# sczhou/ProPainter

Measured on NVIDIA H100. Metric: inpainted frames/sec at 432x240x80f, higher is better.
Workload: dtype f32 (TF32 tensor-core products, fp32 accumulate)

## Files before the change

include/propainter_b200.h:

```cpp
#ifndef PROPAINTER_B200_H
#define PROPAINTER_B200_H
#include <stddef.h>
#include <stdint.h>
#include <cuda_runtime_api.h>

#ifdef __cplusplus
extern "C" {
#endif

#define PP_ABI_VERSION 2
int pp_abi_version(void);
const char* pp_error_string(int code);

int pp_corr_build(const float* fmap, int D, const int* idx1, const int* idx2, int n_pairs, float* lvl0, int h, int w,
                  cudaStream_t stream);
int pp_corr_pool_pyramid(float* const* levels, long planes, int h, int w, cudaStream_t stream);
int pp_corr_lookup(const float* const* levels, const float* coords, float* out, long n_pairs, int h, int w,
                   cudaStream_t stream);
int pp_corr_lookup_ldg(const float* const* levels, const float* coords, float* out, long n_pairs, int h, int w,
                       cudaStream_t stream);
int pp_corr_lookup_f16(const float* const* levels, const float* coords, void* out, int ld_out, long n_pairs, int h, int w,
                       cudaStream_t stream);
int pp_corr_lookup_ldg_f16(const float* const* levels, const float* coords, void* out, int ld_out, long n_pairs, int h, int w,
                           cudaStream_t stream);
// ... 54 lines not shown
int pp_window_mask(const float* pmask, int lt, int h, int w, int fh, int fw, int nwh, int nww, int* flags,
                   cudaStream_t stream);

typedef struct PPAttnParams {
  const float* qkv;
  const float* pool;
  const int* key_tok;
  const int* flags;
  float* out;
  int ld_qkv, ld_pool, ld_out;
  int t, NT, WN, NKO, NP, C;
  int kf_start, kf_step, nkf;
  float scale_log2;
} PPAttnParams;
int pp_sparse_window_attn(const PPAttnParams* prm, int n_windows, cudaStream_t stream);
int pp_sparse_window_attn_mma(const PPAttnParams* prm, int n_windows, cudaStream_t stream);
int pp_sparse_window_attn_f16(const PPAttnParams* prm, int n_windows, cudaStream_t stream);

size_t pp_ffn_overlap_add_workspace_bytes(int frames, int h, int w, int CH);
int pp_ffn_overlap_add(const float* Y, int ldy, float* Z, int ldz, int frames, int h, int w, int CH, void* workspace,
                       size_t ws_bytes, cudaStream_t stream);
int pp_ffn_overlap_add_f16(const void* Y, int ldy, void* Z, int ldz, int frames, int h, int w, int CH, void* workspace,
                           size_t ws_bytes, cudaStream_t stream);

int pp_pool_depthwise(const float* x, int ld_x, const float* w_taps, const float* bias, float* out, int n, int H, int W, int C,
                      int kh, int kw, cudaStream_t stream);
int pp_pool_depthwise_f16(const void* x, int ld_x, const float* w_taps, const float* bias, void* out, int n, int H, int W, int C,
                          int kh, int kw, cudaStream_t stream);
int pp_add_layernorm(const float* x, const float* delta, const float* gamma, const float* beta, float* x_out, float* y, long rows,
                     int C, float eps, cudaStream_t stream);
int pp_add_layernorm_f16(const float* x, const void* delta, int delta_f16, const float* gamma, const float* beta, float* x_out,
                         void* y, int y_f16, long rows, int C, float eps, cudaStream_t stream);

int pp_gru_gate(const float* zr, const float* bias, const float* pre, const float* net, int ld_net, float* z, float* rnet,
                int ld_r, long npix, int C, cudaStream_t stream);
int pp_gru_update(const float* q, const float* bias, const float* pre, const float* z, float* net, int ld_net, float* net_copy,
                  long npix, int C, cudaStream_t stream);
int pp_raft_pack_motion(const float* mot, int ld_mot, const float* bias, const float* flow, float* d0, float* d1, int ld,
                        long npix, cudaStream_t stream);
int pp_gru_gate_f16(const void* zr, const float* bias, const float* pre, const float* net, int ld_net, float* z, void* rnet,
                    int ld_r, long npix, int C, cudaStream_t stream);
int pp_gru_update_f16(const void* q, const float* bias, const float* pre, const float* z, float* net, int ld_net, void* h_img,
                      int ld_img, void* net_copy, long npix, int C, cudaStream_t stream);
int pp_raft_pack_motion_f16(const void* mot, int ld_mot, const float* bias, const float* flow, void* d0, void* d1, int ld,
                            long npix, cudaStream_t stream);
int pp_raft_pack_motion_n(const float* mot, int ld_mot, const float* bias, const float* flow, float* d0, float* d1, int ld,
                          long npix, int cmot, cudaStream_t stream);

int pp_bias_act(const float* x, int ld_x, const float* bias, const float* res, int ld_res, float* out, int ld_out, long n_pix,
                int C, int act, float slope, int post_relu, cudaStream_t stream);
int pp_bias_act_pre(const float* x, int ld_x, const float* bias, const float* pre, int ld_pre, const float* res, int ld_res,
                    float* out, int ld_out, long n_pix, int C, int act, float slope, int post_relu, cudaStream_t stream);
int pp_bias_act_f16(const void* x, int ld_x, int x_f16, const float* bias, const float* pre, int ld_pre, const float* res, int ld_res,
                    void* out, int ld_out, int out_f16, long n_pix, int C, int act, float slope, int post_relu, cudaStream_t stream);

size_t pp_instance_norm_workspace_bytes(int n, long HW, int C);
int pp_instance_norm(const float* x, const float* res, float* out, int n, long HW, int C, float eps, int relu, int post_relu,
                     void* workspace, size_t ws_bytes, cudaStream_t stream);
int pp_upsample2x_bilinear(const float* src, float* dst, int n, int h, int w, int C, cudaStream_t stream);

int pp_mask_dilate(const uint8_t* src, float* dst, int T, int H, int W, int iterations, cudaStream_t stream);
int pp_u8_to_frames(const uint8_t* src, float* dst, int T, int H, int W, cudaStream_t stream);
int pp_resample_coeffs_bicubic(int in_size, int out_size, int* bounds, int* kk, long kk_capacity);
int pp_resample_index_nearest(int in_size, int out_size, int* idx);
int pp_resample_coeffs_linear_cv(int in_size, int out_size, int horizontal, int* ofs, short* coef);
size_t pp_resize_u8_bicubic_workspace_bytes(int T, int H, int Wo);
int pp_resize_u8_bicubic(const uint8_t* src, uint8_t* dst, int T, int H, int W, int Ho, int Wo, const int* bounds_x, const int* kk_x,
                         int ksize_x, const int* bounds_y, const int* kk_y, int ksize_y, void* workspace, size_t ws_bytes,
                         cudaStream_t stream);
int pp_resize_u8_nearest(const uint8_t* src, uint8_t* dst, int T, int H, int W, int Ho, int Wo, int C, const int* idx_x, const int* idx_y,
                         cudaStream_t stream);
int pp_resize_u8_bilinear_cv(const uint8_t* src, uint8_t* dst, int T, int H, int W, int Ho, int Wo, const int* xofs, const short* alpha,
                             const int* yofs, const short* beta, cudaStream_t stream);
int pp_resample_coeffs_linear_f32(int in_size, int out_size, int horizontal, int* ofs, float* coef);
int pp_resize_flow_linear_cv(const float* src, float* dst, int N, int H, int W, int Ho, int Wo, const int* xofs, const float* alpha,
                             const int* yofs, const float* beta, cudaStream_t stream);
#define PP_MAX_WINDOW 32
typedef struct PPWindowIds { int n; int frame[PP_MAX_WINDOW]; int first[PP_MAX_WINDOW]; } PPWindowIds;
int pp_composite_blend_u8(const float* pred, const float* masks, const uint8_t* ori, uint8_t* comp,
                          const PPWindowIds* ids, int H, int W, cudaStream_t stream);
int pp_composite_blend_f32(const float* pred, const float* masks, const uint8_t* ori, float* comp,
                           const PPWindowIds* ids, int H, int W, cudaStream_t stream);
// ... 19 lines not shown
```

propainter_b200/_lib.py:

```python
import ctypes
import os

_HERE = os.path.dirname(os.path.abspath(__file__))
LIB_PATH = os.environ.get("PROPAINTER_B200_LIB") or os.path.join(_HERE, "libpropainter_b200.so")

c_void_p, c_int, c_long, c_float, c_size_t = ctypes.c_void_p, ctypes.c_int, ctypes.c_long, ctypes.c_float, ctypes.c_size_t

PP_MAX_WINDOW = 32


class PPAttnParams(ctypes.Structure):
    _fields_ = [("qkv", c_void_p), ("pool", c_void_p), ("key_tok", c_void_p), ("flags", c_void_p), ("out", c_void_p),
                ("ld_qkv", c_int), ("ld_pool", c_int), ("ld_out", c_int),
                ("t", c_int), ("NT", c_int), ("WN", c_int), ("NKO", c_int), ("NP", c_int), ("C", c_int),
                ("kf_start", c_int), ("kf_step", c_int), ("nkf", c_int), ("scale_log2", c_float)]


PP_CONV_MAX_SEG = 4


class PPConvSeg(ctypes.Structure):
    _fields_ = [("x", c_void_p), ("ld", c_int), ("C", c_int)]


# ... 62 lines not shown
    "pp_gru_update": (c_int, [c_void_p, c_void_p, c_void_p, c_void_p, c_void_p, c_int, c_void_p, c_long, c_int, c_void_p]),
    "pp_raft_pack_motion": (c_int, [c_void_p, c_int, c_void_p, c_void_p, c_void_p, c_void_p, c_int, c_long, c_void_p]),
    "pp_gru_gate_f16": (c_int, [c_void_p, c_void_p, c_void_p, c_void_p, c_int, c_void_p, c_void_p, c_int, c_long, c_int, c_void_p]),
    "pp_gru_update_f16": (c_int, [c_void_p, c_void_p, c_void_p, c_void_p, c_void_p, c_int, c_void_p, c_int, c_void_p, c_long, c_int,
                                  c_void_p]),
    "pp_raft_pack_motion_f16": (c_int, [c_void_p, c_int, c_void_p, c_void_p, c_void_p, c_void_p, c_int, c_long, c_void_p]),
    "pp_raft_pack_motion_n": (c_int, [c_void_p, c_int, c_void_p, c_void_p, c_void_p, c_void_p, c_int, c_long, c_int, c_void_p]),
    "pp_bias_act": (c_int, [c_void_p, c_int, c_void_p, c_void_p, c_int, c_void_p, c_int, c_long, c_int, c_int, c_float, c_int,
                            c_void_p]),
    "pp_bias_act_pre": (c_int, [c_void_p, c_int, c_void_p, c_void_p, c_int, c_void_p, c_int, c_void_p, c_int, c_long, c_int, c_int, c_float,
                                c_int, c_void_p]),
    "pp_bias_act_f16": (c_int, [c_void_p, c_int, c_int, c_void_p, c_void_p, c_int, c_void_p, c_int, c_void_p, c_int, c_int, c_long, c_int,
                                c_int, c_float, c_int, c_void_p]),
    "pp_pool_depthwise": (c_int, [c_void_p, c_int, c_void_p, c_void_p, c_void_p, c_int, c_int, c_int, c_int, c_int, c_int, c_void_p]),
    "pp_add_layernorm": (c_int, [c_void_p, c_void_p, c_void_p, c_void_p, c_void_p, c_void_p, c_long, c_int, c_float, c_void_p]),
    "pp_pool_depthwise_f16": (c_int, [c_void_p, c_int, c_void_p, c_void_p, c_void_p, c_int, c_int, c_int, c_int, c_int, c_int,
                                      c_void_p]),
    "pp_add_layernorm_f16": (c_int, [c_void_p, c_void_p, c_int, c_void_p, c_void_p, c_void_p, c_void_p, c_int, c_long, c_int,
                                     c_float, c_void_p]),
    "pp_instance_norm_workspace_bytes": (c_size_t, [c_int, c_long, c_int]),
    "pp_instance_norm": (c_int, [c_void_p, c_void_p, c_void_p, c_int, c_long, c_int, c_float, c_int, c_int, c_void_p, c_size_t,
                                 c_void_p]),
    "pp_upsample2x_bilinear": (c_int, [c_void_p, c_void_p, c_int, c_int, c_int, c_int, c_void_p]),
    "pp_mask_dilate": (c_int, [c_void_p, c_void_p, c_int, c_int, c_int, c_int, c_void_p]),
    "pp_u8_to_frames": (c_int, [c_void_p, c_void_p, c_int, c_int, c_int, c_void_p]),
    "pp_resample_coeffs_bicubic": (c_int, [c_int, c_int, c_void_p, c_void_p, c_long]),
    "pp_resample_index_nearest": (c_int, [c_int, c_int, c_void_p]),
    "pp_resample_coeffs_linear_cv": (c_int, [c_int, c_int, c_int, c_void_p, c_void_p]),
    "pp_resize_u8_bicubic_workspace_bytes": (c_size_t, [c_int, c_int, c_int]),
    "pp_resize_u8_bicubic": (c_int, [c_void_p, c_void_p, c_int, c_int, c_int, c_int, c_int, c_void_p, c_void_p, c_int, c_void_p, c_void_p,
                                     c_int, c_void_p, c_size_t, c_void_p]),
    "pp_resize_u8_nearest": (c_int, [c_void_p, c_void_p, c_int, c_int, c_int, c_int, c_int, c_int, c_void_p, c_void_p, c_void_p]),
    "pp_resize_u8_bilinear_cv": (c_int, [c_void_p, c_void_p, c_int, c_int, c_int, c_int, c_int, c_void_p, c_void_p, c_void_p, c_void_p,
                                         c_void_p]),
    "pp_composite_blend_u8": (c_int, [c_void_p, c_void_p, c_void_p, c_void_p, ctypes.POINTER(PPWindowIds), c_int, c_int,
                                      c_void_p]),
    "pp_composite_blend_f32": (c_int, [c_void_p, c_void_p, c_void_p, c_void_p, ctypes.POINTER(PPWindowIds), c_int, c_int,
                                       c_void_p]),
    "pp_resample_coeffs_linear_f32": (c_int, [c_int, c_int, c_int, c_void_p, c_void_p]),
    "pp_resize_flow_linear_cv": (c_int, [c_void_p, c_void_p] + [c_int] * 5 + [c_void_p] * 5),
    "pp_extrapolate_u8": (c_int, [c_void_p, c_void_p, c_void_p, c_void_p] + [c_int] * 9 + [c_void_p]),
    "pp_mask_overlay_u8": (c_int, [c_void_p, c_void_p, c_void_p, c_int, c_int, c_int, c_void_p]),
    "pp_flow_maxrad": (c_int, [c_void_p, c_void_p] + [c_int] * 5 + [ctypes.c_float, c_void_p]),
    "pp_flow_to_image_u8": (c_int, [c_void_p, c_void_p, c_void_p] + [c_int] * 5 + [ctypes.c_float, c_int, c_void_p]),
    "pp_i3d_input": (c_int, [c_void_p, c_int, c_void_p, c_int, c_int, c_int, c_int, c_void_p]),
    "pp_maxpool3d_same": (c_int, [c_void_p, c_int, c_void_p, c_int] + [c_int] * 11 + [c_void_p]),
# ... 27 lines not shown
```

propainter_b200/csrc/gather_kernels.cu:

```cuda
#include <stdlib.h>
#include "pp_elem.cuh"
#include "pp_mma.cuh"
#include "../../include/propainter_b200.h"

#define PP_LAUNCH_CHECK() do { if (cudaPeekAtLastError() != cudaSuccess) return PP_ERR_LAUNCH; } while (0)

static inline int pp_blocks(long n, int per) { return (int)((n + per - 1) / per); }

__global__ void __launch_bounds__(256) k_imgprop_step(int H, int W, const float* __restrict__ cur,
    const float* __restrict__ mcur, const float* __restrict__ prev, const float* __restrict__ mprev,
    const float* __restrict__ fprop, const float* __restrict__ fcheck, float* __restrict__ out,
    float* __restrict__ mout, int nearest) {
  int pix = blockIdx.x * blockDim.x + threadIdx.x;
  if (pix < H * W) pp_imgprop_pixel(pix, H, W, cur, mcur, prev, mprev, fprop, fcheck, out, mout, nearest);
}

extern "C" size_t pp_img_prop_scan_workspace_bytes(int t, int H, int W) {
  return (size_t)t * 4 * H * W * sizeof(float);
}

extern "C" int pp_img_prop_scan(const float* frames, const float* flows_f, const float* flows_b,
                                const float* masks, float* out_frames, float* out_masks, void* workspace,
                                size_t ws_bytes, int t, int H, int W, int nearest, cudaStream_t stream) {
  if (t < 1 || H < 2 || W < 2) return PP_ERR_SHAPE;
// ... 412 lines not shown
  if (ws_bytes < pp_ffn_overlap_add_workspace_bytes(frames, h, w, CH)) return PP_ERR_WORKSPACE;
  float* F = (float*)workspace;
  const long n1 = (long)h * w * (CH / 4), n2 = (long)fh * fw * 49 * (CH / 4);
  if (n2 > 0x7fffffffL) return PP_ERR_SHAPE;
  k_ffn_fold_gelu<T><<<dim3(pp_blocks(n1, 256), frames), 256, 0, stream>>>(Y, ldy, CH, fh, fw, h, w, F);
  k_ffn_unfold<T><<<dim3(pp_blocks(n2, 256), frames), 256, 0, stream>>>(F, CH, fh, fw, h, w, Z, ldz);
  PP_LAUNCH_CHECK();
  return PP_OK;
}
extern "C" int pp_ffn_overlap_add(const float* Y, int ldy, float* Z, int ldz, int frames, int h, int w, int CH,
                                  void* workspace, size_t ws_bytes, cudaStream_t stream) {
  if (ldy < 49 * CH || ldz < 49 * CH || frames < 1 || frames > 65535) return PP_ERR_SHAPE;
  if (CH % 4 || ldy % 4 || ldz % 4) return PP_ERR_ALIGN;
  return pp_ffn_launch(Y, ldy, Z, ldz, frames, h, w, CH, workspace, ws_bytes, stream);
}
extern "C" int pp_ffn_overlap_add_f16(const void* Y, int ldy, void* Z, int ldz, int frames, int h, int w, int CH,
                                      void* workspace, size_t ws_bytes, cudaStream_t stream) {
  if (ldy < 49 * CH || ldz < 49 * CH || frames < 0 || frames > 65535) return PP_ERR_SHAPE;
  if (CH % 4 || ldy % 8 || ldz % 8 || ((uintptr_t)Y & 15) || ((uintptr_t)Z & 15) || ((uintptr_t)workspace & 15)) return PP_ERR_ALIGN;
  if (frames == 0 || h <= 0 || w <= 0) return PP_OK;
  return pp_ffn_launch((const __half*)Y, ldy, (__half*)Z, ldz, frames, h, w, CH, workspace, ws_bytes, stream);
}

template <typename TX, typename TO>
__global__ void __launch_bounds__(256) k_bias_act(const TX* x, int ld_x, const float* __restrict__ bias, const float* res,
                                                  int ld_res, TO* out, int ld_out, long n_pix, int C, int act, float slope,
                                                  int post_relu, const float* __restrict__ pre = nullptr, int ld_pre = 0) {
  const int c4n = C >> 2;
  const long i = (long)blockIdx.x * blockDim.x + threadIdx.x;
  if (i >= n_pix * c4n) return;
  const long pix = i / c4n; const int c = (int)(i - pix * c4n) * 4;
  const float4 v = pp_ld4(x + pix * ld_x + c);
  float r[4] = {v.x, v.y, v.z, v.w};
  if (bias != nullptr) {
    const float4 b = *reinterpret_cast<const float4*>(bias + c);
    r[0] += b.x; r[1] += b.y; r[2] += b.z; r[3] += b.w;
  }
  if (pre != nullptr) {
    const float4 b = *reinterpret_cast<const float4*>(pre + pix * ld_pre + c);
    r[0] += b.x; r[1] += b.y; r[2] += b.z; r[3] += b.w;
  }
#pragma unroll
  for (int k = 0; k < 4; ++k) {
    float t = r[k];
    if (act == 1) t = fmaxf(t, 0.f);
    else if (act == 2) t = t > 0.f ? t : t * slope;
// ... 135 lines not shown
#pragma unroll
      for (int e = 0; e < 4; ++e) y[e] = fmaxf(y[e], 0.f);
    }
    *reinterpret_cast<float4*>(out + off) = make_float4(y[0], y[1], y[2], y[3]);
  }
}
extern "C" size_t pp_instance_norm_workspace_bytes(int n, long HW, int C) {
  return (size_t)n * pp_in_splits(n, HW) * 2 * C * sizeof(float);
}
extern "C" int pp_instance_norm(const float* x, const float* res, float* out, int n, long HW, int C, float eps, int relu,
                                int post_relu, void* workspace, size_t ws_bytes, cudaStream_t stream) {
  if (C % 4 || ((uintptr_t)x & 15) || ((uintptr_t)out & 15) || ((uintptr_t)res & 15) || ((uintptr_t)workspace & 15)) return PP_ERR_ALIGN;
  if (C < 4 || C > 512 || n < 1 || n > 65535 || HW < 1) return PP_ERR_SHAPE;
  if (ws_bytes < pp_instance_norm_workspace_bytes(n, HW, C)) return PP_ERR_WORKSPACE;
  const int S = pp_in_splits(n, HW);
  const int chunk = (int)((HW + S - 1) / S);
  float* part = (float*)workspace;
  k_inorm_stats<<<dim3(S, n), 256, 0, stream>>>(x, HW, C, chunk, S, part);
  k_inorm_apply<<<dim3(S, n), 256, 0, stream>>>(x, part, S, res, out, HW, C, chunk, eps, relu, post_relu);
  PP_LAUNCH_CHECK();
  return PP_OK;
}

__global__ void __launch_bounds__(256) k_upsample2x(const float* __restrict__ src, float* __restrict__ dst, int n, int h,
                                                    int w, int C) {
  const int c4n = C >> 2, H = 2 * h, W = 2 * w;
  const long i = (long)blockIdx.x * blockDim.x + threadIdx.x;
  if (i >= (long)n * H * W * c4n) return;
  const int c = (int)(i % c4n) * 4; const long px = i / c4n;
  const int b = (int)(px / ((long)H * W)); const int r = (int)(px - (long)b * H * W); const int y = r / W, x = r - y * W;
  const PPUp uy = pp_up2_coord(y, h), ux = pp_up2_coord(x, w);
  const float* p = src + (((long)b * h + uy.i0) * w + ux.i0) * C + c;
  const float4 v00 = *reinterpret_cast<const float4*>(p), v01 = *reinterpret_cast<const float4*>(p + (long)ux.step * C);
  const float4 v10 = *reinterpret_cast<const float4*>(p + (long)uy.step * w * C);
  const float4 v11 = *reinterpret_cast<const float4*>(p + ((long)uy.step * w + ux.step) * C);
  float4 o;
  o.x = pp_up2_blend(v00.x, v01.x, v10.x, v11.x, uy, ux); o.y = pp_up2_blend(v00.y, v01.y, v10.y, v11.y, uy, ux);
  o.z = pp_up2_blend(v00.z, v01.z, v10.z, v11.z, uy, ux); o.w = pp_up2_blend(v00.w, v01.w, v10.w, v11.w, uy, ux);
  reinterpret_cast<float4*>(dst)[i] = o;
}
extern "C" int pp_upsample2x_bilinear(const float* src, float* dst, int n, int h, int w, int C, cudaStream_t stream) {
  if (C % 4) return PP_ERR_ALIGN;
  if (h < 2 || w < 2) return PP_ERR_SHAPE;
  const long total = (long)n * 4 * h * w * (C / 4);
  k_upsample2x<<<pp_blocks(total, 256), 256, 0, stream>>>(src, dst, n, h, w, C);
  PP_LAUNCH_CHECK();
  return PP_OK;
}

template <typename T>
__global__ void __launch_bounds__(256) k_gru_gate(const T* __restrict__ zr, const float* __restrict__ bias,
    const float* __restrict__ pre, const float* __restrict__ net, int ld_net, float* __restrict__ z, T* __restrict__ rnet,
    int ld_r, long npix, int C) {
  const int c4n = C >> 2;
  const long i = (long)blockIdx.x * blockDim.x + threadIdx.x;
  if (i >= npix * c4n) return;
  const long pix = i / c4n; const int c = (int)(i - pix * c4n) * 4;
  float4 zv = pp_ld4(zr + pix * 2 * C + c), rv = pp_ld4(zr + pix * 2 * C + C + c);
  float4 bz = make_float4(0.f, 0.f, 0.f, 0.f), br = bz;
  if (bias != nullptr) { bz = *reinterpret_cast<const float4*>(bias + c); br = *reinterpret_cast<const float4*>(bias + C + c); }
  if (pre != nullptr) {
    const float4 pz = *reinterpret_cast<const float4*>(pre + pix * 2 * C + c), pr = *reinterpret_cast<const float4*>(pre + pix * 2 * C + C + c);
    zv.x += pz.x; zv.y += pz.y; zv.z += pz.z; zv.w += pz.w; rv.x += pr.x; rv.y += pr.y; rv.z += pr.z; rv.w += pr.w;
  }
  const float4 h = *reinterpret_cast<const float4*>(net + pix * ld_net + c);
  float4 zo, ro;
  zo.x = 1.0f / (1.0f + expf(-(zv.x + bz.x))); zo.y = 1.0f / (1.0f + expf(-(zv.y + bz.y)));
  zo.z = 1.0f / (1.0f + expf(-(zv.z + bz.z))); zo.w = 1.0f / (1.0f + expf(-(zv.w + bz.w)));
// ... 445 lines not shown
```

propainter_b200/model/modules/sparse_transformer.py:

```python
import torch
import torch.nn.functional as F

from ... import config, ops
from ...nn_util import as_nchw, as_pm, cl, conv
from ...window_index import padded_grid, token_grid, window_key_table

WIN = (5, 9)
POOL = (4, 4)
KS, ST, PD = 7, 3, 3


class TransformerExec:
    def __init__(self, net, depths=8, hidden=512, channel=128, ffn_ch=40):
        self.net, self.depths, self.hidden, self.channel, self.ffn_ch = net, depths, hidden, channel, ffn_ch

    def _ss(self):
        def build():
            P = self.net.P
            return cl(P["ss.embedding.weight"].view(self.hidden, self.channel, KS, KS)), P["ss.embedding.bias"].contiguous()
        return self.net.packed("ss", build)

    def _sc(self):
        def build():
            P = self.net.P
            w = P["sc.embedding.weight"].view(self.channel, KS, KS, self.hidden).permute(3, 0, 1, 2).contiguous()
            return w
# ... 16 lines not shown
            wpool = P[p + "pool_layer.weight"]
            return w, b, wkv, bkv, wpool.reshape(wpool.shape[0], -1).t().contiguous(), P[p + "pool_layer.bias"].contiguous()
        return self.net.packed(f"qkv{i}", build)

    def _ffn(self, i):
        def build():
            P, p = self.net.P, f"transformers.transformer.{i}.mlp."
            ch = self.ffn_ch
            perm = torch.arange(49 * ch, device=P[p + "fc1.0.weight"].device).view(ch, 49).t().reshape(-1)
            return (P[p + "fc1.0.weight"][perm].contiguous(), P[p + "fc1.0.bias"][perm].contiguous(),
                    P[p + "fc2.1.weight"][:, perm].contiguous(), P[p + "fc2.1.bias"].contiguous())
        return self.net.packed(f"ffn{i}", build)

    def _qkv_half(self, i):
        return self.net.packed(f"f16:qkv{i}", lambda: tuple(t.half() for t in self._qkv(i)[:4]) + self._qkv(i)[4:])

    def _proj_half(self, i):
        P, p = self.net.P, f"transformers.transformer.{i}.attention.proj."
        return self.net.packed(f"f16:proj{i}", lambda: (P[p + "weight"].half(), P[p + "bias"].half()))

    def _ffn_half(self, i):
        return self.net.packed(f"f16:ffn{i}", lambda: tuple(t.half() for t in self._ffn(i)))

    def soft_split(self, feat):
        return as_pm(conv(feat, self._ss(), ST, PD))

    def soft_comp(self, tokens, hw, res=None):
        fh, fw = tokens.shape[1:3]
        op = (hw[0] + 2 - 3 * fh, hw[1] + 2 - 3 * fw)
        y = F.conv_transpose2d(as_nchw(tokens), self._sc(), None, stride=ST, padding=PD, output_padding=op)
        y = y + self._sc_bias_map(tuple(hw))
        P = self.net.P
        return conv(y, self.net.packed("scbc", lambda: (cl(P["sc.bias_conv.weight"]), P["sc.bias_conv.bias"].contiguous())), 1, 1,
                    res=res)

    def run(self, tokens, hw, flags, t_dilation=2):
        assert self.depths % t_dilation == 0, "wrong t_dilation input."
        with config.linear_precision():
            if tokens.is_cuda and config.half_linears():
                with config.fp32_reductions():
                    return self._run(tokens, hw, flags, t_dilation, True)
            return self._run(tokens, hw, flags, t_dilation, False)

    def _run(self, tokens, hw, flags, t_dilation, half):
        t, fh, fw, C = tokens.shape
        H2, W2 = padded_grid(fh, fw, WIN)
        NT = H2 * W2
        key_tok = self.net.packed(f"ktab:{H2}x{W2}", lambda: torch.from_numpy(window_key_table(H2, W2, WIN)).to(tokens.device))
        P = self.net.P
        x = tokens.contiguous()
        pad = (H2 != fh) or (W2 != fw)
        norm = lambda i, k: (P[f"transformers.transformer.{i}.norm{k}.weight"], P[f"transformers.transformer.{i}.norm{k}.bias"])
        yd = {"y_dtype": torch.float16} if half else {}
        _, y = ops.add_layernorm(x, None, *norm(0, 1), **yd)
        for i in range(self.depths):
            p = f"transformers.transformer.{i}."
            wqkv, bqkv, wkv, bkv, wpool, bpool = self._qkv_half(i) if half else self._qkv(i)
# ... 21 lines not shown
```

propainter_b200/model/propainter.py:

```python
import torch
import torch.nn.functional as F

from .. import autotune, config, ops
from .._params import ParamNet
from ..graphs import high_priority
from ..nn_util import as_nchw, as_pm, cl, conv, pad_in_channels, up2
from ..schemas import generator_schema
from ..window_index import padded_grid, token_grid
from .modules.sparse_transformer import WIN, TransformerExec


def _flow_in(f):
    return f.contiguous() if f.dtype == torch.float16 else f.contiguous().float()


def _lrelu(x, s=0.2):
    return F.leaky_relu_(x, s)


class InpaintGenerator(ParamNet):
    def __init__(self, init_weights=True, model_path=None, seed=None):
        super().__init__(generator_schema(), seed=seed)
        self.tx = TransformerExec(self)
        if model_path is not None:
# ... 52 lines not shown

            def grouped(x0, o, key=key, g=g):
                mix = torch.cat([x0.view(n, h, w, g, -1), o.view(n, h, w, g, -1)], -1).view(n, h, w, -1)
                return conv(as_nchw(mix), self._wb(key), 1, 1, 1, g, **L)

            def per_group(x0, o, key=key, g=g):
                a, b = x0.shape[-1] // g, o.shape[-1] // g
                co = self.P[key + ".weight"].shape[0] // g
                res = torch.empty(n, h, w, g * co, device=x0.device)
                for j in range(g):
                    xin = torch.cat([x0[..., j * a:(j + 1) * a], o[..., j * b:(j + 1) * b]], -1)
                    conv(as_nchw(xin), self._wb_group(key, j, g), 1, 1, out=as_nchw(res[..., j * co:(j + 1) * co]), **L)
                return as_nchw(res)

            o = as_pm(out)
            if g == 1:
                out = grouped(x0, o)
            else:
                out = autotune.pick(("enc_group", i, tuple(x0.shape), tuple(o.shape)), (grouped, per_group), x0, o)
        return out

    def _decoder(self, x):
        L = dict(act="leaky", slope=0.2)
        x = conv(up2(x), self._wb("decoder.0.conv"), 1, 1, **L)
        x = conv(x, self._wb("decoder.2"), 1, 1, **L)
        x = conv(up2(x), self._wb("decoder.4.conv"), 1, 1, **L)
        return conv(x, self._wb("decoder.6"), 1, 1)

    def _feat_propagation(self, x, dsf, dsb, pmask, interpolation, gather_gemm=False):
        if interpolation != "bilinear":
            raise NotImplementedError("the feature propagation path uses bilinear warping (propainter.py:319 default)")
        lt, h, w, C = x.shape
        dev = x.device
        fp = "feat_prop_module."
        cond = torch.empty(1, h, w, 2 * C + 8, device=dev)
        bb = torch.empty(1, h, w, 2 * C + 4, device=dev)
        src = x
        outs = {}
        for name in ("backward_1", "forward_1"):
            bwd = name == "backward_1"
            order = list(range(lt))[::-1] if bwd else list(range(lt))
            dst = torch.empty(lt, h, w, C, device=dev)
            dw, db = self._dcn(name)
            if gather_gemm:
                dwp = self.packed("dcnu:" + name, lambda: ops.pack_deform_weight_umma(self.P[f"{fp}deform_align.{name}.weight"]))
                cols = torch.empty(1, h, w, 9 * C, device=dev)
            prev = None
            for i, idx in enumerate(order):
                if i == 0:
                    ops.prop_cond(src[idx], None, None, None, pmask[idx], None, bb[0], True)
# ... 197 lines not shown
        fh, fw = token_grid((h, w))
        H2, W2 = padded_grid(fh, fw, WIN)
        flags = ops.window_mask(pmask, fh, fw, H2 // WIN[0], W2 // WIN[1])
        enc_pm = as_pm(enc)
        if interpolation != "bilinear":
            raise NotImplementedError("the feature propagation path uses bilinear warping (propainter.py:319 default)")
        xl = enc_pm[:lt]

        def scan():
            if config.UMMA_CONV == "auto":
                return autotune.pick(("gen_prop", tuple(xl.shape[1:])), (lambda a, b, c, d: self._feat_propagation_umma(a, b, c, d),
                                                                          lambda a, b, c, d: self._feat_propagation(a, b, c, d, interpolation),
                                                                          lambda a, b, c, d: self._feat_propagation(a, b, c, d, interpolation, True),
                                                                          lambda a, b, c, d: self._feat_propagation_hoisted(a, b, c, d)),
                                     xl, dsf, dsb, pmask, reps=2, graph_timed=True)
            if config.UMMA_CONV == "hoisted":
                return self._feat_propagation_hoisted(xl, dsf, dsb, pmask)
            if config.UMMA_CONV == "hybrid":
                return self._feat_propagation(xl, dsf, dsb, pmask, interpolation, True)
            if config.UMMA_CONV:
                return self._feat_propagation_umma(xl, dsf, dsb, pmask)
            return self._feat_propagation(xl, dsf, dsb, pmask, interpolation)
        local = high_priority(scan)
        enc2 = torch.cat([local, enc[lt:]], 0).contiguous(memory_format=torch.channels_last)
        tok_in = self.tx.soft_split(enc2)
        tok = self.tx.run(tok_in, (h, w), flags, t_dilation)
        enc3 = self.tx.soft_comp(tok, (h, w), res=enc2)
        if parts is not None:
            parts.update(prop_feat=local.contiguous(), tokens_in=tok_in, tokens_out=tok, enc_out=enc3.contiguous())
        return torch.tanh(self._decoder(enc3[:lt])).contiguous()
```

propainter_b200/ops.py:

```python
import collections
import ctypes
import math

import torch

from . import _lib
from ._lib import PPAttnParams, PPConvParams, PPWindowIds, check

LOG2E = 1.4426950408889634

LAUNCHES = 0


def _count(n):
    global LAUNCHES
    LAUNCHES += n


def _stream():
    return ctypes.c_void_p(torch.cuda.current_stream().cuda_stream)


def _p(t, dtype=torch.float32):
    if t is None:
# ... 463 lines not shown
        check(_lib.lib().pp_bias_act_f16(xp, ldx, int(x_pm.dtype == torch.float16), _p(bias), pp, ldp, rp, ldr, op, ldo,
                                         int(out.dtype == torch.float16), x_pm.numel() // C, C, ACT[act], float(slope),
                                         int(bool(post_relu)), _stream()), "pp_bias_act_f16")
        _count(1)
        return out
    xp, ldx = _pm(x_pm)
    op, ldo = _pm(out)
    rp, ldr = _pm(res) if res is not None else (None, C)
    if pre is not None:
        pp, ldp = _pm(pre)
        check(_lib.lib().pp_bias_act_pre(xp, ldx, _p(bias), pp, ldp, rp, ldr, op, ldo, x_pm.numel() // C, C, ACT[act], float(slope),
                                         int(bool(post_relu)), _stream()), "pp_bias_act_pre")
    else:
        check(_lib.lib().pp_bias_act(xp, ldx, _p(bias), rp, ldr, op, ldo, x_pm.numel() // C, C, ACT[act], float(slope),
                                     int(bool(post_relu)), _stream()), "pp_bias_act")
    _count(1)
    return out


def bias_act_(x_pm, bias, act="none", slope=0.0):
    return bias_act(x_pm, bias, act, slope)


def pool_depthwise(x_pm, w_taps, bias, kh, kw):
    n, H, W, C = x_pm.shape
    xp, ld = _pm(x_pm, x_pm.dtype)
    out = torch.empty(n, (H - kh) // kh + 1, (W - kw) // kw + 1, C, device=x_pm.device, dtype=x_pm.dtype)
    fn, name = ((_lib.lib().pp_pool_depthwise_f16, "pp_pool_depthwise_f16") if x_pm.dtype == torch.float16 else
                (_lib.lib().pp_pool_depthwise, "pp_pool_depthwise"))
    check(fn(xp, ld, _p(_dense(w_taps)), _p(bias), _p(out, x_pm.dtype), n, H, W, C, kh, kw, _stream()), name)
    _count(1)
    return out


def add_layernorm(x, delta, gamma, beta, eps=1e-5, y_dtype=torch.float32):
    C = x.shape[-1]
    y = torch.empty_like(x, dtype=y_dtype)
    xo = torch.empty_like(x) if delta is not None else None
    if torch.float16 in (y_dtype, delta.dtype if delta is not None else None):
        dt = delta.dtype if delta is not None else torch.float32
        check(_lib.lib().pp_add_layernorm_f16(_p(_dense(x)), _p(_dense(delta), dt) if delta is not None else None,
                                              int(dt == torch.float16), _p(gamma), _p(beta), _p(xo), _p(y, y_dtype),
                                              int(y_dtype == torch.float16), x.numel() // C, C, float(eps), _stream()),
              "pp_add_layernorm_f16")
        _count(1)
        return (xo if delta is not None else x), y
    check(_lib.lib().pp_add_layernorm(_p(_dense(x)), _p(_dense(delta)) if delta is not None else None, _p(gamma), _p(beta),
                                      _p(xo), _p(y), x.numel() // C, C, float(eps), _stream()), "pp_add_layernorm")
    _count(1)
    return (xo if delta is not None else x), y


def instance_norm(x_pm, relu=False, res=None, post_relu=False, eps=1e-5, out=None):
    n, h, w, C = x_pm.shape
    out = torch.empty_like(x_pm) if out is None else out
    lib = _lib.lib()
    nbytes = lib.pp_instance_norm_workspace_bytes(n, h * w, C)
    ws = torch.empty(max(nbytes // 4, 4), device=x_pm.device, dtype=torch.float32)
    check(lib.pp_instance_norm(_p(_dense(x_pm)), _p(_dense(res)) if res is not None else None, _p(_dense(out)), n, h * w, C,
                               float(eps), int(bool(relu)), int(bool(post_relu)), _p(ws), ws.numel() * 4, _stream()),
          "pp_instance_norm")
    _count(2)
    return out


def upsample2x(x_pm):
    n, h, w, C = x_pm.shape
    out = torch.empty(n, 2 * h, 2 * w, C, device=x_pm.device, dtype=torch.float32)
    check(_lib.lib().pp_upsample2x_bilinear(_p(_dense(x_pm)), _p(out), n, h, w, C, _stream()), "pp_upsample2x_bilinear")
    _count(1)
    return out


def mask_dilate(masks_u8, iterations):
    T, H, W = masks_u8.shape
    out = torch.empty(T, 1, H, W, device=masks_u8.device, dtype=torch.float32)
    check(_lib.lib().pp_mask_dilate(_p(_dense(masks_u8), torch.uint8), _p(out), T, H, W, int(iterations), _stream()),
          "pp_mask_dilate")
    _count(1)
    return out


def u8_to_frames(frames_u8):
    T, H, W, _ = frames_u8.shape
    out = torch.empty(T, 3, H, W, device=frames_u8.device, dtype=torch.float32)
    check(_lib.lib().pp_u8_to_frames(_p(_dense(frames_u8), torch.uint8), _p(out), T, H, W, _stream()), "pp_u8_to_frames")
    _count(1)
    return out


def composite_blend(pred, masks, ori_u8, comp_u8, frame_ids, first_flags):
    n, _, H, W = pred.shape
# ... 224 lines not shown
```

Measured before the change: 223.5.

## Run transformer trunk soft split/comp and decoder in fp16 with fold kernel

Adds an fp16 path for the SoftSplit conv, SoftComp (either conv_transpose or a GEMM plus a custom fold kernel, picked by autotune), the bias conv and the decoder convs, including a new fp16 bilinear upsample kernel. SoftComp now computes only the local frames instead of all frames. The goal is to cut the memory traffic and tensor-core time of the trunk convolutions. Everything depends on config.half_convs/HALF_OPERANDS being enabled, and it brings fp16 accuracy risk.

```diff
diff --git a/include/propainter_b200.h b/include/propainter_b200.h
--- a/include/propainter_b200.h
+++ b/include/propainter_b200.h
@@ -100,6 +100,7 @@
                        size_t ws_bytes, cudaStream_t stream);
 int pp_ffn_overlap_add_f16(const void* Y, int ldy, void* Z, int ldz, int frames, int h, int w, int CH, void* workspace,
                            size_t ws_bytes, cudaStream_t stream);
+int pp_sc_fold_f16(const void* cols, long ldc, const float* bmap, void* out, int frames, int h, int w, int C, cudaStream_t stream);
 
 int pp_pool_depthwise(const float* x, int ld_x, const float* w_taps, const float* bias, float* out, int n, int H, int W, int C,
                       int kh, int kw, cudaStream_t stream);
@@ -136,6 +137,7 @@
 int pp_instance_norm(const float* x, const float* res, float* out, int n, long HW, int C, float eps, int relu, int post_relu,
                      void* workspace, size_t ws_bytes, cudaStream_t stream);
 int pp_upsample2x_bilinear(const float* src, float* dst, int n, int h, int w, int C, cudaStream_t stream);
+int pp_upsample2x_bilinear_f16(const void* src, void* dst, int n, int h, int w, int C, cudaStream_t stream);
 
 int pp_mask_dilate(const uint8_t* src, float* dst, int T, int H, int W, int iterations, cudaStream_t stream);
 int pp_u8_to_frames(const uint8_t* src, float* dst, int T, int H, int W, cudaStream_t stream);
diff --git a/profiles/half_trunk_time.py b/profiles/half_trunk_time.py
--- /dev/null
+++ b/profiles/half_trunk_time.py
@@ -0,0 +1,153 @@
+import os
+import statistics
+import subprocess
+import sys
+
+import torch
+import torch.nn.functional as F
+
+ROOT = os.path.dirname(os.path.dirname(os.path.abspath(__file__)))
+sys.path.insert(0, ROOT)
+import __graft_entry__ as g
+
+g.build()
+from bench import WORKLOADS
+from propainter_b200 import config, ops, synth
+from propainter_b200.inference_propainter import InferenceConfig, ProPainterPipeline
+
+wl = WORKLOADS[sys.argv[1] if len(sys.argv) > 1 else "c2"]
+reps = int(sys.argv[2]) if len(sys.argv) > 2 else 5
+modes = (False, True)
+try:
+    card = subprocess.run(["nvidia-smi", "--query-gpu=name,power.limit,clocks.max.sm", "--format=csv,noheader"],
+                          capture_output=True, text=True).stdout.strip()
+except OSError:
+    card = "nvidia-smi unavailable"
+print("card:", card, "|", torch.cuda.get_device_name(0))
+
+u8, fm, md = synth.make_clip(wl["T"], wl["H"], wl["W"], mask=wl["mask"], seed=0)
+u8d, fmd, mdd = torch.from_numpy(u8).cuda(), fm.cuda(), md.cuda()
+pipe = ProPainterPipeline(device="cuda")
+cfg = InferenceConfig(raft_iter=wl["raft_iter"])
+inputs = {}
+with torch.no_grad():
+    for m in modes:
+        config.HALF_OPERANDS = m
+        frames = ops.u8_to_frames(u8d).unsqueeze(0)
+        pred = pipe.complete_flows(pipe.compute_flows(frames, cfg), fmd, cfg)
+        inputs[m] = pipe.propagate_images(frames, mdd, pred, cfg), pred
+torch.cuda.synchronize()
+
+
+def stage4(m):
+    config.HALF_OPERANDS = m
+    upd, pred = inputs[m]
+    e0, e1 = torch.cuda.Event(enable_timing=True), torch.cuda.Event(enable_timing=True)
+    with torch.no_grad():
+        e0.record()
+        pipe.generate(upd[0], mdd, upd[1], pred, u8d, cfg)
+        e1.record()
+    torch.cuda.synchronize()
+    return e0.elapsed_time(e1)
+
+
+for m in modes:
+    for _ in range(2):
+        stage4(m)
+runs = {m: [] for m in modes}
+for _ in range(reps):
+    for m in modes:
+        runs[m].append(stage4(m))
+for m in modes:
+    v = runs[m]
+    print(f"HALF_OPERANDS={m}: stage 4 ms over {reps} reps (min / median / max) {min(v):8.2f} {statistics.median(v):8.2f} {max(v):8.2f}")
+
+from torch.profiler import ProfilerActivity, profile
+
+for m in modes:
+    config.HALF_OPERANDS = m
+    upd, pred = inputs[m]
+    with torch.no_grad(), profile(activities=[ProfilerActivity.CUDA]) as prof:
+        pipe.generate(upd[0], mdd, upd[1], pred, u8d, cfg)
+        torch.cuda.synchronize()
+    print(f"\nHALF_OPERANDS={m}: stage 4 kernels")
+    print(prof.key_averages().table(sort_by="cuda_time_total", row_limit=30, max_name_column_width=90))
+
+t, lt, h, w, C, HID = 18, 11, 60, 108, 128, 512
+fh, fw = (h - 1) // 3 + 1, (w - 1) // 3 + 1
+flush = torch.empty(256 << 20, dtype=torch.uint8, device="cuda")
+torch.backends.cudnn.allow_tf32 = True
+torch.backends.cudnn.benchmark = True
+torch.backends.cuda.matmul.allow_tf32 = True
+torch.backends.cuda.matmul.allow_fp16_reduced_precision_reduction = False
+
+
+def timed(fn, n=20):
+    fn()
+    ts = []
+    for _ in range(n):
+        flush.zero_()
+        e0, e1 = torch.cuda.Event(enable_timing=True), torch.cuda.Event(enable_timing=True)
+        e0.record()
+        fn()
+        e1.record()
+        torch.cuda.synchronize()
+        ts.append(e0.elapsed_time(e1))
+    return statistics.median(ts)
+
+
+def cl4(*shape, dt):
+    return torch.randn(*shape, device="cuda").to(dt).contiguous(memory_format=torch.channels_last)
+
+
+def report(name, flop, fn, dt):
+    ms = timed(fn)
+    peak = 989 if dt == torch.float16 else 495
+    tf = flop / (ms * 1e-3) / 1e12
+    print(f"  {name:34s} {str(dt):14s} {ms:7.3f} ms {tf:7.1f} TFLOP/s ({100 * tf / peak:.0f} % of {peak})")
+    return ms
+
+
+print(f"\ntrunk ops at the C2 window shape (t = {t}, lt = {lt}, {h} x {w} features, {fh} x {fw} tokens), median of 20, L2 flushed")
+for dt in (torch.float32, torch.float16):
+    s = 0.0
+    x = cl4(t, C, h, w, dt=dt)
+    wss = cl4(HID, C, 7, 7, dt=dt) / 80
+    s += report("SoftSplit conv 7x7/s3 128->512, t", 2 * t * fh * fw * HID * C * 49, lambda: F.conv2d(x, wss, None, 3, 3), dt)
+    tok = cl4(t, HID, fh, fw, dt=dt)
+    wsc = torch.randn(HID, C, 7, 7, device="cuda").to(dt) / 23
+    for n in (t, lt):
+        s_ = report(f"SoftComp conv_transpose2d, {n} frames", 2 * n * fh * fw * HID * C * 49,
+                    lambda: F.conv_transpose2d(tok[:n], wsc, None, 3, 3, (h + 2 - 3 * fh, w + 2 - 3 * fw)), dt)
+    s += s_
+    if dt == torch.float16:
+        tok2 = torch.randn(lt * fh * fw, HID, device="cuda").half()
+        wcol = torch.randn(49 * C, HID, device="cuda").half() / 23
+        bmap = torch.randn(h, w, C, device="cuda")
+        cols = torch.empty(lt * fh * fw, 49 * C, device="cuda", dtype=dt)
+        fold_out = torch.empty(lt, h, w, C, device="cuda", dtype=dt)
+        report(f"SoftComp GEMM (fold plan), {lt} frames", 2 * lt * fh * fw * HID * C * 49, lambda: torch.mm(tok2, wcol.t(), out=cols), dt)
+        ms = timed(lambda: ops.sc_fold(cols, bmap, lt, h, w, out=fold_out))
+        nbytes = cols.numel() * 2 + bmap.numel() * 4 + fold_out.numel() * 2
+        print(f"  {'SoftComp fold kernel, ' + str(lt) + ' frames':34s} {str(dt):14s} {ms:7.3f} ms {nbytes / (ms * 1e-3) / 1e9:7.1f} GB/s "
+              f"({100 * nbytes / (ms * 1e-3) / 3.35e12:.0f} % of 3.35 TB/s)")
+    wbc = cl4(C, C, 3, 3, dt=dt) / 34
+    s += report(f"sc.bias_conv 3x3 128->128, {lt} frames", 2 * lt * h * w * C * C * 9, lambda: F.conv2d(x[:lt], wbc, None, 1, 1), dt)
+    d0 = cl4(lt, C, 2 * h, 2 * w, dt=dt)
+    w0 = cl4(64, C, 3, 3, dt=dt) / 34
+    s += report("decoder.0 3x3 128->64 @120x216", 2 * lt * 4 * h * w * 64 * C * 9, lambda: F.conv2d(d0, w0, None, 1, 1), dt)
+    d2 = cl4(lt, 64, 2 * h, 2 * w, dt=dt)
+    w2 = cl4(64, 64, 3, 3, dt=dt) / 24
+    s += report("decoder.2 3x3 64->64 @120x216", 2 * lt * 4 * h * w * 64 * 64 * 9, lambda: F.conv2d(d2, w2, None, 1, 1), dt)
+    d4 = cl4(lt, 64, 4 * h, 4 * w, dt=dt)
+    s += report("decoder.4 3x3 64->64 @240x432", 2 * lt * 16 * h * w * 64 * 64 * 9, lambda: F.conv2d(d4, w2, None, 1, 1), dt)
+    w6 = cl4(3, 64, 3, 3, dt=dt) / 24
+    w6p = cl4(4, 64, 3, 3, dt=dt) / 24
+    s += report("decoder.6 3x3 64->3 @240x432", 2 * lt * 16 * h * w * 3 * 64 * 9, lambda: F.conv2d(d4, w6, None, 1, 1), dt)
+    report("decoder.6 padded to 64->4", 2 * lt * 16 * h * w * 4 * 64 * 9, lambda: F.conv2d(d4, w6p, None, 1, 1), dt)
+    print(f"  {'library convs above, summed':34s} {str(dt):14s} {s:7.3f} ms per window, {16 * s:7.2f} ms per 16 windows")
+    for name, src in (("upsample2x 128 ch @60x108", torch.randn(lt, h, w, C, device="cuda").to(dt)),
+                      ("upsample2x 64 ch @120x216", torch.randn(lt, 2 * h, 2 * w, 64, device="cuda").to(dt))):
+        ms = timed(lambda: ops.upsample2x(src))
+        nbytes = src.numel() * src.element_size() * 5
+        print(f"  {name:34s} {str(dt):14s} {ms:7.3f} ms {nbytes / (ms * 1e-3) / 1e9:7.1f} GB/s ({100 * nbytes / (ms * 1e-3) / 3.35e12:.0f} % of 3.35 TB/s)")
diff --git a/propainter_b200/_lib.py b/propainter_b200/_lib.py
--- a/propainter_b200/_lib.py
+++ b/propainter_b200/_lib.py
@@ -108,6 +108,8 @@
     "pp_instance_norm": (c_int, [c_void_p, c_void_p, c_void_p, c_int, c_long, c_int, c_float, c_int, c_int, c_void_p, c_size_t,
                                  c_void_p]),
     "pp_upsample2x_bilinear": (c_int, [c_void_p, c_void_p, c_int, c_int, c_int, c_int, c_void_p]),
+    "pp_upsample2x_bilinear_f16": (c_int, [c_void_p, c_void_p, c_int, c_int, c_int, c_int, c_void_p]),
+    "pp_sc_fold_f16": (c_int, [c_void_p, c_long, c_void_p, c_void_p, c_int, c_int, c_int, c_int, c_void_p]),
     "pp_mask_dilate": (c_int, [c_void_p, c_void_p, c_int, c_int, c_int, c_int, c_void_p]),
     "pp_u8_to_frames": (c_int, [c_void_p, c_void_p, c_int, c_int, c_int, c_void_p]),
     "pp_resample_coeffs_bicubic": (c_int, [c_int, c_int, c_void_p, c_void_p, c_long]),
diff --git a/propainter_b200/csrc/gather_kernels.cu b/propainter_b200/csrc/gather_kernels.cu
--- a/propainter_b200/csrc/gather_kernels.cu
+++ b/propainter_b200/csrc/gather_kernels.cu
@@ -458,6 +458,37 @@
   return pp_ffn_launch((const __half*)Y, ldy, (__half*)Z, ldz, frames, h, w, CH, workspace, ws_bytes, stream);
 }
 
+template <typename T>
+__global__ void __launch_bounds__(256) k_sc_fold(const T* __restrict__ cols, long ldc, const float* __restrict__ bmap, int C,
+                                                 int fh, int fw, int h, int w, T* __restrict__ out) {
+  const int c4n = C >> 2;
+  const int i = blockIdx.x * blockDim.x + threadIdx.x;
+  if (i >= h * w * c4n) return;
+  const int c = (i % c4n) * 4, px = i / c4n, y = px / w, x = px - y * w;
+  const T* cf = cols + (long)blockIdx.y * fh * fw * ldc;
+  float4 s = make_float4(0.f, 0.f, 0.f, 0.f);
+  for (int ty = (y + 3) / 3, ky; ty >= 0 && (ky = y + 3 - 3 * ty) < 7; --ty) {
+    if (ty >= fh) continue;
+    for (int tx = (x + 3) / 3, kx; tx >= 0 && (kx = x + 3 - 3 * tx) < 7; --tx) {
+      if (tx >= fw) continue;
+      const float4 v = pp_ld4(cf + (long)(ty * fw + tx) * ldc + (ky * 7 + kx) * C + c);
+      s.x += v.x; s.y += v.y; s.z += v.z; s.w += v.w;
+    }
+  }
+  const float4 b = *reinterpret_cast<const float4*>(bmap + (long)px * C + c);
+  pp_st4(out + ((long)blockIdx.y * h * w + px) * C + c, make_float4(s.x + b.x, s.y + b.y, s.z + b.z, s.w + b.w));
+}
+extern "C" int pp_sc_fold_f16(const void* cols, long ldc, const float* bmap, void* out, int frames, int h, int w, int C,
+                              cudaStream_t stream) {
+  if (frames < 0 || frames > 65535 || h < 1 || w < 1 || C < 4 || ldc < 49L * C || (long)h * w * C > 0x7fffffffL) return PP_ERR_SHAPE;
+  if (C % 4 || ldc % 4 || ((uintptr_t)cols & 7) || ((uintptr_t)out & 7) || ((uintptr_t)bmap & 15)) return PP_ERR_ALIGN;
+  if (frames == 0) return PP_OK;
+  k_sc_fold<__half><<<dim3(pp_blocks((long)h * w * (C / 4), 256), frames), 256, 0, stream>>>(
+      (const __half*)cols, ldc, bmap, C, (h - 1) / 3 + 1, (w - 1) / 3 + 1, h, w, (__half*)out);
+  PP_LAUNCH_CHECK();
+  return PP_OK;
+}
+
 template <typename TX, typename TO>
 __global__ void __launch_bounds__(256) k_bias_act(const TX* x, int ld_x, const float* __restrict__ bias, const float* res,
                                                   int ld_res, TO* out, int ld_out, long n_pix, int C, int act, float slope,
@@ -639,28 +670,41 @@
   return PP_OK;
 }
 
-__global__ void __launch_bounds__(256) k_upsample2x(const float* __restrict__ src, float* __restrict__ dst, int n, int h,
-                                                    int w, int C) {
-  const int c4n = C >> 2, H = 2 * h, W = 2 * w;
+template <typename T>
+__global__ void __launch_bounds__(256) k_upsample2x(const T* __restrict__ src, T* __restrict__ dst, int n, int h, int w, int C) {
+  constexpr int V = 16 / sizeof(T);
+  const int cvn = C >> (V == 4 ? 2 : 3), H = 2 * h, W = 2 * w;
   const long i = (long)blockIdx.x * blockDim.x + threadIdx.x;
-  if (i >= (long)n * H * W * c4n) return;
-  const int c = (int)(i % c4n) * 4; const long px = i / c4n;
+  if (i >= (long)n * H * W * cvn) return;
+  const int c = (int)(i % cvn) * V; const long px = i / cvn;
   const int b = (int)(px / ((long)H * W)); const int r = (int)(px - (long)b * H * W); const int y = r / W, x = r - y * W;
   const PPUp uy = pp_up2_coord(y, h), ux = pp_up2_coord(x, w);
-  const float* p = src + (((long)b * h + uy.i0) * w + ux.i0) * C + c;
-  const float4 v00 = *reinterpret_cast<const float4*>(p), v01 = *reinterpret_cast<const float4*>(p + (long)ux.step * C);
-  const float4 v10 = *reinterpret_cast<const float4*>(p + (long)uy.step * w * C);
-  const float4 v11 = *reinterpret_cast<const float4*>(p + ((long)uy.step * w + ux.step) * C);
-  float4 o;
-  o.x = pp_up2_blend(v00.x, v01.x, v10.x, v11.x, uy, ux); o.y = pp_up2_blend(v00.y, v01.y, v10.y, v11.y, uy, ux);
-  o.z = pp_up2_blend(v00.z, v01.z, v10.z, v11.z, uy, ux); o.w = pp_up2_blend(v00.w, v01.w, v10.w, v11.w, uy, ux);
-  reinterpret_cast<float4*>(dst)[i] = o;
+  const T* p = src + (((long)b * h + uy.i0) * w + ux.i0) * C + c;
+#pragma unroll
+  for (int k = 0; k < V; k += 4) {
+    const float4 v00 = pp_ld4(p + k), v01 = pp_ld4(p + (long)ux.step * C + k);
+    const float4 v10 = pp_ld4(p + (long)uy.step * w * C + k);
+    const float4 v11 = pp_ld4(p + ((long)uy.step * w + ux.step) * C + k);
+    float4 o;
+    o.x = pp_up2_blend(v00.x, v01.x, v10.x, v11.x, uy, ux); o.y = pp_up2_blend(v00.y, v01.y, v10.y, v11.y, uy, ux);
+    o.z = pp_up2_blend(v00.z, v01.z, v10.z, v11.z, uy, ux); o.w = pp_up2_blend(v00.w, v01.w, v10.w, v11.w, uy, ux);
+    pp_st4(dst + i * V + k, o);
+  }
 }
 extern "C" int pp_upsample2x_bilinear(const float* src, float* dst, int n, int h, int w, int C, cudaStream_t stream) {
   if (C % 4) return PP_ERR_ALIGN;
   if (h < 2 || w < 2) return PP_ERR_SHAPE;
   const long total = (long)n * 4 * h * w * (C / 4);
-  k_upsample2x<<<pp_blocks(total, 256), 256, 0, stream>>>(src, dst, n, h, w, C);
+  k_upsample2x<float><<<pp_blocks(total, 256), 256, 0, stream>>>(src, dst, n, h, w, C);
+  PP_LAUNCH_CHECK();
+  return PP_OK;
+}
+extern "C" int pp_upsample2x_bilinear_f16(const void* src, void* dst, int n, int h, int w, int C, cudaStream_t stream) {
+  if (C % 8 || ((uintptr_t)src & 15) || ((uintptr_t)dst & 15)) return PP_ERR_ALIGN;
+  if (n < 0 || h < 2 || w < 2) return PP_ERR_SHAPE;
+  if (n == 0) return PP_OK;
+  const long total = (long)n * 4 * h * w * (C / 8);
+  k_upsample2x<__half><<<pp_blocks(total, 256), 256, 0, stream>>>((const __half*)src, (__half*)dst, n, h, w, C);
   PP_LAUNCH_CHECK();
   return PP_OK;
 }
diff --git a/propainter_b200/model/modules/sparse_transformer.py b/propainter_b200/model/modules/sparse_transformer.py
--- a/propainter_b200/model/modules/sparse_transformer.py
+++ b/propainter_b200/model/modules/sparse_transformer.py
@@ -1,7 +1,7 @@
 import torch
 import torch.nn.functional as F
 
-from ... import config, ops
+from ... import autotune, config, ops
 from ...nn_util import as_nchw, as_pm, cl, conv
 from ...window_index import padded_grid, token_grid, window_key_table
 
@@ -64,17 +64,54 @@
     def _ffn_half(self, i):
         return self.net.packed(f"f16:ffn{i}", lambda: tuple(t.half() for t in self._ffn(i)))
 
+    def _ss_half(self):
+        return self.net.packed("f16:ss", lambda: (self._ss()[0].half(), self._ss()[1]))
+
+    def _sc_half(self):
+        def build():
+            W = self.net.P["sc.embedding.weight"]
+            wcol = W.view(self.channel, KS * KS, self.hidden).transpose(0, 1).reshape(-1, self.hidden)
+            return self._sc().half(), wcol.half().contiguous()
+        return self.net.packed("f16:sc", build)
+
+    def _scbc(self, half):
+        P = self.net.P
+        wb = self.net.packed("scbc", lambda: (cl(P["sc.bias_conv.weight"]), P["sc.bias_conv.bias"].contiguous()))
+        return self.net.packed("f16:scbc", lambda: (wb[0].half(), wb[1])) if half else wb
+
     def soft_split(self, feat):
+        if feat.dtype == torch.float16:
+            t, _, h, w = feat.shape
+            fh, fw = token_grid((h, w))
+            out = torch.empty(t, fh, fw, self.hidden, device=feat.device)
+            conv(feat, self._ss_half(), ST, PD, out=as_nchw(out))
+            return out
         return as_pm(conv(feat, self._ss(), ST, PD))
 
-    def soft_comp(self, tokens, hw, res=None):
+    def soft_comp(self, tokens, hw, res, frames, half=False, out_dtype=torch.float32):
         fh, fw = tokens.shape[1:3]
-        op = (hw[0] + 2 - 3 * fh, hw[1] + 2 - 3 * fw)
-        y = F.conv_transpose2d(as_nchw(tokens), self._sc(), None, stride=ST, padding=PD, output_padding=op)
-        y = y + self._sc_bias_map(tuple(hw))
-        P = self.net.P
-        return conv(y, self.net.packed("scbc", lambda: (cl(P["sc.bias_conv.weight"]), P["sc.bias_conv.bias"].contiguous())), 1, 1,
-                    res=res)
+        tok = tokens[:frames]
+        bmap = self._sc_bias_map(tuple(hw))
+        if not half:
+            op = (hw[0] + 2 - 3 * fh, hw[1] + 2 - 3 * fw)
+            y = F.conv_transpose2d(as_nchw(tok), self._sc(), None, stride=ST, padding=PD, output_padding=op)
+            y = y + bmap
+        else:
+            tok16 = tok.half()
+            wt, wcol = self._sc_half()
+
+            def tconv(tok16):
+                op = (hw[0] + 2 - 3 * fh, hw[1] + 2 - 3 * fw)
+                y = F.conv_transpose2d(as_nchw(tok16), wt, None, stride=ST, padding=PD, output_padding=op)
+                return torch.add(y, bmap, out=torch.empty_like(y))
+
+            def fold(tok16):
+                with config.fp32_reductions():
+                    cols = torch.mm(tok16.view(-1, self.hidden), wcol.t())
+                return as_nchw(ops.sc_fold(cols, as_pm(bmap)[0], frames, hw[0], hw[1]))
+            y = autotune.pick(("sc_half", tuple(tok16.shape), tuple(hw)), (fold, tconv), tok16)
+        out = torch.empty(frames, hw[0], hw[1], self.channel, device=tokens.device, dtype=out_dtype)
+        return conv(y, self._scbc(half), 1, 1, res=res, out=as_nchw(out))
 
     def run(self, tokens, hw, flags, t_dilation=2):
         assert self.depths % t_dilation == 0, "wrong t_dilation input."
diff --git a/propainter_b200/model/propainter.py b/propainter_b200/model/propainter.py
--- a/propainter_b200/model/propainter.py
+++ b/propainter_b200/model/propainter.py
@@ -98,10 +98,20 @@
 
     def _decoder(self, x):
         L = dict(act="leaky", slope=0.2)
-        x = conv(up2(x), self._wb("decoder.0.conv"), 1, 1, **L)
-        x = conv(x, self._wb("decoder.2"), 1, 1, **L)
-        x = conv(up2(x), self._wb("decoder.4.conv"), 1, 1, **L)
-        return conv(x, self._wb("decoder.6"), 1, 1)
+        if x.dtype != torch.float16:
+            x = conv(up2(x), self._wb("decoder.0.conv"), 1, 1, **L)
+            x = conv(x, self._wb("decoder.2"), 1, 1, **L)
+            x = conv(up2(x), self._wb("decoder.4.conv"), 1, 1, **L)
+            return conv(x, self._wb("decoder.6"), 1, 1)
+        wb16 = lambda k: self.packed("f16:" + k, lambda: (self._wb(k)[0].half(), self._wb(k)[1]))
+        x = conv(up2(x), wb16("decoder.0.conv"), 1, 1, **L)
+        x = conv(x, wb16("decoder.2"), 1, 1, **L)
+        x = conv(up2(x), wb16("decoder.4.conv"), 1, 1, **L)
+        w6, b6 = self.packed("f16:decoder.6", lambda: (cl(F.pad(self.P["decoder.6.weight"], (0, 0, 0, 0, 0, 0, 0, 1))).half(),
+                                                       F.pad(self.P["decoder.6.bias"], (0, 1)).contiguous()))
+        n, _, H, W = x.shape
+        out = torch.empty(n, H, W, 4, device=x.device)
+        return conv(x, (w6, b6), 1, 1, out=as_nchw(out))[:, :3]
 
     def _feat_propagation(self, x, dsf, dsb, pmask, interpolation, gather_gemm=False):
         if interpolation != "bilinear":
@@ -345,10 +355,22 @@
                 return self._feat_propagation_umma(xl, dsf, dsb, pmask)
             return self._feat_propagation(xl, dsf, dsb, pmask, interpolation)
         local = high_priority(scan)
-        enc2 = torch.cat([local, enc[lt:]], 0).contiguous(memory_format=torch.channels_last)
+        half = enc.is_cuda and config.half_convs()
+        if half:
+            t = enc.shape[0]
+            enc2 = torch.empty(t, h, w, enc.shape[1], device=enc.device, dtype=torch.float16)
+            enc2[:lt].copy_(as_pm(local))
+            enc2[lt:].copy_(enc_pm[lt:])
+            enc2 = as_nchw(enc2)
+        else:
+            enc2 = torch.cat([local, enc[lt:]], 0).contiguous(memory_format=torch.channels_last)
         tok_in = self.tx.soft_split(enc2)
         tok = self.tx.run(tok_in, (h, w), flags, t_dilation)
-        enc3 = self.tx.soft_comp(tok, (h, w), res=enc2)
-        if parts is not None:
+        if parts is None:
+            enc3 = self.tx.soft_comp(tok, (h, w), local, lt, half, torch.float16 if half else torch.float32)
+        else:
+            res = torch.cat([local, enc[lt:]], 0).contiguous(memory_format=torch.channels_last)
+            enc3 = self.tx.soft_comp(tok, (h, w), res, enc.shape[0], half)
             parts.update(prop_feat=local.contiguous(), tokens_in=tok_in, tokens_out=tok, enc_out=enc3.contiguous())
-        return torch.tanh(self._decoder(enc3[:lt])).contiguous()
+            enc3 = enc3[:lt].half() if half else enc3[:lt]
+        return torch.tanh(self._decoder(enc3)).contiguous()
diff --git a/propainter_b200/ops.py b/propainter_b200/ops.py
--- a/propainter_b200/ops.py
+++ b/propainter_b200/ops.py
@@ -509,6 +509,20 @@
     return bias_act(x_pm, bias, act, slope)
 
 
+def sc_fold(cols, bmap, frames, h, w, out=None):
+    C = bmap.shape[-1]
+    fh, fw = (h - 1) // 3 + 1, (w - 1) // 3 + 1
+    if cols.dim() != 2 or cols.shape[0] != frames * fh * fw or cols.stride(1) != 1 or tuple(bmap.shape) != (h, w, C):
+        raise RuntimeError("sc_fold: shape mismatch")
+    out = torch.empty(frames, h, w, C, device=cols.device, dtype=torch.float16) if out is None else out
+    if tuple(out.shape) != (frames, h, w, C):
+        raise RuntimeError("sc_fold: out shape mismatch")
+    check(_lib.lib().pp_sc_fold_f16(_p(cols, torch.float16), cols.stride(0), _p(_dense(bmap)), _p(_dense(out), torch.float16), frames,
+                                    h, w, C, _stream()), "pp_sc_fold_f16")
+    _count(1)
+    return out
+
+
 def pool_depthwise(x_pm, w_taps, bias, kh, kw):
     n, H, W, C = x_pm.shape
     xp, ld = _pm(x_pm, x_pm.dtype)
@@ -553,8 +567,12 @@
 
 def upsample2x(x_pm):
     n, h, w, C = x_pm.shape
-    out = torch.empty(n, 2 * h, 2 * w, C, device=x_pm.device, dtype=torch.float32)
-    check(_lib.lib().pp_upsample2x_bilinear(_p(_dense(x_pm)), _p(out), n, h, w, C, _stream()), "pp_upsample2x_bilinear")
+    out = torch.empty(n, 2 * h, 2 * w, C, device=x_pm.device, dtype=x_pm.dtype)
+    if x_pm.dtype == torch.float16:
+        check(_lib.lib().pp_upsample2x_bilinear_f16(_p(_dense(x_pm), torch.float16), _p(out, torch.float16), n, h, w, C, _stream()),
+              "pp_upsample2x_bilinear_f16")
+    else:
+        check(_lib.lib().pp_upsample2x_bilinear(_p(_dense(x_pm)), _p(out), n, h, w, C, _stream()), "pp_upsample2x_bilinear")
     _count(1)
     return out
 
```

Result: faster. 237.4, median of 6 (+6.2%).
